# raphaelsulzer/PixelsPointsPolygons

Measured on AMD Instinct MI355X. Metric: training tiles/sec (224px img + 3k-pt lidar), higher is better.
Workload: dtype f32 (products as bf16x3 on the bf16 MFMA, fp32 accumulate); 1 GPU; pix2poly_fusion_s8_bs64x1; tiles_per_gpu=64, points_per_tile=3000, hip_graph=True, sync_bn=False, decoder_dropout=reference defaults (0.1 / 0.05), step=fwd+CE+10*BCE+bwd+AdamW, parallelism=dp1

## Files before the change

### include/p3hip.h

```cpp
#ifndef P3HIP_H
#define P3HIP_H
#include <stdint.h>

#ifdef __cplusplus
extern "C" {
#endif

#define P3_OK 0
#define P3_EINVAL (-1)
#define P3_ESHAPE (-2)
#define P3_EALIGN (-3)
#define P3_EUNSUP (-4)

#define P3_F32 0
#define P3_BF16 1
#define P3_F32X3 2

#define P3_ACT_NONE 0
#define P3_ACT_GELU 1
#define P3_ACT_RELU 2
#define P3_ACT_MUL 3
#define P3_ACT_BN_RELU 4

#define P3_A_PLAIN 0
// ... 217 lines not shown
int p3_gemm_tn(const void* A, const void* B, float* C, int M, int N, int K, int lda, int ldb, int ldc, int dtype, void* stream);
int p3_colsum(const void* x, float* out, int64_t M, int N, int ld, int dtype, void* stream);
int p3_act_bwd(const void* dy, int dtype_dy, const void* saved, int dtype_saved, void* out, int dtype_out, int64_t n, int act, float scale,
               void* stream);
int p3_embed_tokens_bwd(const void* dx, int dtype, const int64_t* tokens, float* demb, float* dpos, int B, int L, int D, void* stream);
int p3_embed_tokens_bwd_v(const void* dx, int dtype, const int64_t* tokens, float* demb, int B, int L, int D, int V, void* stream);
int p3_tokens_assemble_bwd(const float* dx, const void* src, int src_ld, int dtype_src, const float* scale, const float* shift, const float* mean,
                           void* dsrc, float* dscale, float* dshift, int B, int np, int D, void* stream);
int p3_pool_pos_bwd(const void* dout, int dtype_dout, void* dy, int dtype_dy, int B, int np, int Din, int Dout, void* stream);
int p3_pair_mean_bwd(const float* dF, void* dfeats, int dtype, int B, int L, int N, int D, int accumulate, void* stream);
int p3_sinkhorn_bwd(const float* scores, const float* alpha, int B, int m, int n, int iters, const float* perm,
                    const float* uv_hist, const float* dperm, float* dscores, float* dalpha, void* workspace, void* stream);
int64_t p3_sinkhorn_bwd_workspace_bytes(int B, int m, int n, int iters);
int p3_ce_loss_fwd(const float* logits, int ld, const int64_t* targets, int R, int V, int ignore_index, float* row_lse, float* acc, void* stream);
int p3_ce_loss_bwd(const float* logits, int ld, const int64_t* targets, int R, int V, int ignore_index, const float* row_lse,
                   const float* acc, const float* gscale, void* dlogits, int dtype_out, int ld_out, int Vpad, void* stream);
int p3_bce_loss_fwd(const float* p, const float* y, int64_t n, float* acc, void* stream);
int p3_bce_loss_bwd(const float* p, const float* y, int64_t n, const float* gscale, float* dp, void* stream);
int p3_adamw_schedule(long long* step, float* hyper, float base_lr, int kind, int warmup_steps, int total_steps, float beta1, float beta2,
                      void* stream);
int p3_adamw_schedule_dev(long long* step, float* hyper, const float* sched, float beta1, float beta2, void* stream);
int p3_adamw(float* params, const float* grads, float* exp_avg, float* exp_avg_sq, int64_t n, const float* hyper, float beta1,
             float beta2, float eps, float weight_decay, float grad_scale, void* bf16_shadow, void* stream);

int p3_gemm_tn_ex(const void* A, const void* B, float* C, int M, int N, int K, int lda, int ldb, int ldc, int dtype, int b_mode,
                  const float* b_scale, const float* b_shift, const void* pair_V, int pair_n, float* colsum ,
                  float* slabs ,
                  int max_slabs, void* stream);
int p3_row_affine_bwd(const void* dA, const float* dS, const void* H, const float* scale, const float* shift, const float* mean, const float* w4,
                      void* dHd, float* acc, int64_t R, int C, int N, int transpose, int dtype, void* stream);
int p3_row_affine_bwd2(const void* dA, const float* dS, const void* H, const float* scale, const float* shift, const float* mean,
                       const float* w4, void* dHd, float* acc, const float* fix_a, const float* fix_b, int64_t R, int C, int N,
                       int transpose, int dtype, void* stream);
int p3_bn_bwd_coeffs(const float* dscale, const float* dshift, const float* gamma, const float* mean, const float* rstd, float count,
                     int training, int C, float* dgamma, float* dbeta, float* a, float* b, void* stream);
int p3_affine_fix(void* dH, const void* H, const float* a, const float* b, int64_t R, int C, int dtype, void* stream);
int p3_affine_fix_ld(void* dH, const void* H, int ldh, const float* a, const float* b, int64_t R, int C, int dtype, void* stream);
int p3_pair_bwd(const void* dA, const void* U, const void* V, const float* scale, const float* shift, const float* mean, float* dU, float* dV, float* acc,
                int B, int N, int C, int dtype, void* stream);
int64_t p3_pair_bwd_workspace_bytes(int B, int N, int C);
int64_t p3_pair_bwd_workspace_bytes_dt(int B, int N, int C, int dtype);
int p3_pair_bwd_ws(const void* dA, const void* U, const void* V, const float* scale, const float* shift, const float* mean, float* dU, float* dV,
                   float* acc, int B, int N, int C, int dtype, void* workspace, void* stream);
int p3_bn_sums_from_g(const float* G, int ldg, const float* W, const float* scale, const float* shift, const float* mean, float* dW, float* acc,
                      int N, int K, void* stream);
int64_t p3_pair_bwd_fused_workspace_bytes(int B, int N);
int p3_pair_bwd_fused(const void* dH2, const void* W2t, const void* U, const void* V, const float* scale, const float* shift, const float* mean,
                      float* dU, float* dV, float* acc, int B, int N, void* workspace, void* stream);
int p3_pair_stats_bwd(const void* U, const void* V, const float* a, const float* b, float* dU, float* dV, int B, int N, int C, int dtype,
                      void* stream);
int p3_pair_bwd_fused_x3(const float* dH2, const float* W2t, const float* U, const float* V, const float* scale, const float* shift, const float* mean,
                         float* dU, float* dV, float* acc, int B, int N, void* workspace, void* stream);

int p3_upsample_bilinear(const void* src, int dtype_src, void* dst, int dtype_dst, int B, int h, int w, int C, int H, int W, int ld,
                         int src_tok_off, int src_tok_per_img, void* stream);
int p3_head1x1(const void* X, int ld, int dtype, const float* scale, const float* shift, const float* W, const float* bias, int n_out,
               int act, float post_mul, float* out_nchw, void* copy_dst, int copy_ld, int64_t R, int64_t HW, void* stream);
int p3_nhwc_to_nchw(const void* X, int ld, int dtype, const float* scale, const float* shift, float* out, int B, int C, int64_t HW, void* stream);

int p3_head1x1_bwd(const void* H, int dtype, const float* scale, const float* shift, const float* mean, const float* W, int n_out,
                   const float* out_nchw, const float* dout_nchw, int act, float post_mul, void* dHd, float* acc, int64_t R, int64_t HW,
                   void* stream);
int p3_affine_relu_bwd256(const void* dA, const void* H, int ldh, int dtype, const float* scale, const float* shift, const float* mean,
                          void* dHd, float* acc, int64_t R, void* stream);
int p3_pad_nhwc(const void* src, int ld_src, int dtype, const float* scale, const float* shift, int c_aff, int C, int Cp, void* dst, int B, int H,
                int W, void* stream);
// ... 81 lines not shown
```

### pixelspointspolygons_amd/backward.py

```python
import torch

SUMS_FROM_G = [__import__("os").environ.get("P3_SUMS_FROM_G", "1") != "0"]
FUSED_BN2 = [__import__("os").environ.get("P3_BN2_FUSED", "1") != "0"]
FUSED_PAIR = [__import__("os").environ.get("P3_PAIR_FUSED", "1") != "0"]


def scorenet_backward(net, feats, keep, dout, transpose_acc):
    from . import ops
    return ops.drive_steps([scorenet_backward_steps(net, feats, keep, dout, transpose_acc)])[0]


def scorenet_backward_steps(net, feats, keep, dout, transpose_acc):
    from . import hip, ops
    cd, N, training = net.cd, net.n_vertices, net.training
    B, L, D = feats.shape
    dev = feats.device
    R = B * N * N
    F_, U, V, H2, H3 = keep["F"], keep["U"], keep["V"], keep["H2"], keep["H3"]
    (sc1, sh1, m1, r1), (sc2, sh2, m2, r2), (sc3, sh3, m3, r3) = keep["bn"]
    cnt = float(R)
    w2d = lambda conv: conv.weight.reshape(conv.weight.shape[0], -1)
    f32 = dict(dtype=torch.float32, device=dev)
    acc3 = torch.zeros(3 * 64 + 1, **f32)
    dS, w4 = dout.contiguous(), net.conv4.weight.detach().reshape(-1)
    dH3 = hip.row_affine_bwd(H3, sc3, sh3, m3, acc3, dS=dS, w4=w4, N=N, transpose=transpose_acc, store=not training)
    dw4, db4 = acc3[128:192].view(1, 64, 1, 1), acc3[192:193]
    dg3, dbt3, a3, b3 = yield from ops.bn_backward_coeffs_steps(acc3[:64], acc3[64:128], net.bn3.weight.detach(), m3, r3, cnt, training, params=(net.bn3.weight, net.bn3.bias))
    if training:
        dH3 = hip.row_affine_bwd(H3, sc3, sh3, m3, None, dS=dS, w4=w4, N=N, transpose=transpose_acc, fix=(a3, b3))
    gw = {n: ops.direct_grads(getattr(net, n).weight) for n in ("conv1", "conv2", "conv3")}
    wout = lambda n, r, c: gw[n][0].view(r, c) if gw[n] is not None else torch.zeros(r, c, **f32)
    db3 = ops.bias_grad_before_bn(dH3, training, net.conv3.bias)
    w3t = ops.shadow(net.conv3.weight, cd, key="2dT", fn=lambda t: t.reshape(t.shape[0], -1).t())
    acc2 = torch.zeros(2 * 128, **f32)
    fused2 = training and SUMS_FROM_G[0] and FUSED_BN2[0]
    dA3 = None if fused2 else hip.gemm(dH3, w3t, out_dtype=cd)
    if training and SUMS_FROM_G[0]:
        G = torch.zeros((64, 256), **f32)
        hip.gemm_tn_ex(dH3, H2, G, hip.A_AFFINE_MASK2, sc2, sh2)
        dW3 = wout("conv3", 64, 128)
        hip.bn_sums_from_g(G, net.conv3.weight.detach().reshape(64, 128), sc2, sh2, m2, dW3, acc2)
        dH2 = None
    else:
        dW3 = hip.gemm_tn_ex(dH3, H2, wout("conv3", 64, 128), hip.A_AFFINE_RELU, sc2, sh2)
        dH2 = hip.row_affine_bwd(H2, sc2, sh2, m2, acc2, dA=dA3, out=dA3, store=not training)
    dg2, dbt2, a2, b2 = yield from ops.bn_backward_coeffs_steps(acc2[:128], acc2[128:], net.bn2.weight.detach(), m2, r2, cnt, training, params=(net.bn2.weight, net.bn2.bias))
    if fused2:
        dH2 = hip.gemm(dH3, w3t, out_dtype=cd, bwd=(H2, hip.ACT_BN_RELU, torch.stack([sc2, sh2, a2, b2])))
    elif training:
        dH2 = hip.row_affine_bwd(H2, sc2, sh2, m2, None, dA=dA3, out=dA3, fix=(a2, b2))
    dW2 = hip.gemm_tn_ex(dH2, U, wout("conv2", 128, 256), hip.A_PAIR_AFFINE_RELU, sc1, sh1, pair_v=V, pair_n=N, M=R)
    db2 = ops.bias_grad_before_bn(dH2, training, net.conv2.bias)
    w2t = ops.shadow(net.conv2.weight, cd, key="2dT", fn=lambda t: t.reshape(t.shape[0], -1).t())
    acc1 = torch.zeros(2 * 256, **f32)
    if (cd == torch.bfloat16 or (cd == torch.float32 and hip.split_now())) and FUSED_PAIR[0]:
        dU, dV = hip.pair_bwd_fused(dH2, w2t, U, V, sc1, sh1, m1, B, N, acc1)
    else:
        dA2 = hip.gemm(dH2, w2t, out_dtype=cd)
        dU, dV = hip.pair_bwd(dA2, U, V, sc1, sh1, m1, B, N, acc1)
    dg1, dbt1, a1, b1 = yield from ops.bn_backward_coeffs_steps(acc1[:256], acc1[256:], net.bn1.weight.detach(), m1, r1, cnt, training, params=(net.bn1.weight, net.bn1.bias))
    if training:
        hip.pair_stats_bwd(U, V, a1, b1, dU, dV, B, N)
    dUc, dVc = hip.cast(dU, cd), hip.cast(dV, cd)
    F2 = F_.view(B * N, D)
    dW1 = wout("conv1", 256, 2 * D)
    hip.gemm_tn(dUc, F2, out=dW1[:, :D])
    hip.gemm_tn(dVc, F2, out=dW1[:, D:])
    db1 = ops.bias_grad_before_bn(dU, training, net.conv1.bias)
    w1t = ops.shadow(net.conv1.weight, cd, key="2dT2", fn=lambda t: torch.cat([t.reshape(256, -1)[:, :D].t(), t.reshape(256, -1)[:, D:].t()], 0))
    dF = hip.gemm(dUc, w1t[:D], out_dtype=torch.float32)
    dF = hip.gemm(dVc, w1t[D:], out_dtype=torch.float32, residual=dF)
    dfeats = hip.pair_mean_bwd(dF, B, L, N, D, feats.dtype)
    wret = lambda n, t, shape: None if gw[n] is not None else t.view(*shape)
    if any(v is not None for v in gw.values()):
        ops._grad_ready(*(getattr(net, n).weight for n in gw if gw[n] is not None))
    grads = {"conv1.weight": wret("conv1", dW1, (256, 2 * D, 1, 1)), "conv1.bias": db1, "bn1.weight": dg1, "bn1.bias": dbt1,
             "conv2.weight": wret("conv2", dW2, (128, 256, 1, 1)), "conv2.bias": db2, "bn2.weight": dg2, "bn2.bias": dbt2,
             "conv3.weight": wret("conv3", dW3, (64, 128, 1, 1)), "conv3.bias": db3, "bn3.weight": dg3, "bn3.bias": dbt3,
             "conv4.weight": dw4, "conv4.bias": db4}
    return dfeats, [grads[n] for n, _ in net.named_parameters()]
```

### pixelspointspolygons_amd/csrc/mask2_dw_x3.hip

```cpp
#include <stdlib.h>

#include "p3_common.h"

namespace {

constexpr int MX_ROWS = 64;
constexpr int MX_A = MX_ROWS * 128, MX_B = MX_ROWS * 256;
constexpr int MX_OFF_AL = MX_A, MX_OFF_M1 = 2 * MX_A, MX_OFF_M2H = MX_OFF_M1 + MX_B, MX_OFF_M2L = MX_OFF_M2H + MX_B;
constexpr int MX_STEP = MX_OFF_M2L + MX_B;
constexpr int MX_LDS = 2 * MX_STEP;

struct MxArgs {
    const float* dH; const float* H2; const float* sc; const float* sh;
    float* C; int ldc; float* slabs; int64_t steps;
};

__global__ __launch_bounds__(512, 2) void mask2_dw_x3_kernel(MxArgs g) {
    extern __shared__ __attribute__((aligned(1024))) unsigned char lds[];
    const int tid = threadIdx.x, lane = tid & 63, wave = __builtin_amdgcn_readfirstlane(tid >> 6), l31 = lane & 31;
    const int mi = wave & 1, nq = wave >> 1;
    const uint32_t lds_addr = __builtin_amdgcn_readfirstlane((uint32_t)(uintptr_t)lds);
    const int64_t my_steps = (g.steps - (int64_t)blockIdx.x + (int64_t)gridDim.x - 1) / (int64_t)gridDim.x;
    const int ar = tid >> 3, ack = tid & 7, bck = tid & 15;
    float scv[8], shv[8];
#pragma unroll
    for (int e = 0; e < 8; ++e) { scv[e] = g.sc[bck * 8 + e]; shv[e] = g.sh[bck * 8 + e]; }
    float4 pa[2], pb[2][2];
    auto fetch = [&](int64_t q) __attribute__((always_inline)) {
        const int64_t row0 = ((int64_t)blockIdx.x + q * (int64_t)gridDim.x) * MX_ROWS;
        const float* ap = g.dH + (row0 + ar) * 64 + ack * 8;
        pa[0] = *reinterpret_cast<const float4*>(ap); pa[1] = *reinterpret_cast<const float4*>(ap + 4);
#pragma unroll
        for (int k = 0; k < 2; ++k) {
            const float* bp = g.H2 + (row0 + k * 32 + (tid >> 4)) * 128 + bck * 8;
            pb[k][0] = *reinterpret_cast<const float4*>(bp); pb[k][1] = *reinterpret_cast<const float4*>(bp + 4);
        }
    };
    auto commit = [&](int buf) __attribute__((always_inline)) {
        unsigned char* base = lds + buf * MX_STEP;
        {
            const float x[8] = {pa[0].x, pa[0].y, pa[0].z, pa[0].w, pa[1].x, pa[1].y, pa[1].z, pa[1].w};
            u32x4_t h, l;
            split8(x, h, l);
            const uint32_t off = (uint32_t)(ar * 128 + ((ack ^ (((ar >> 1) & 1) << 2)) * 16));
            *reinterpret_cast<u32x4_t*>(base + off) = h;
            *reinterpret_cast<u32x4_t*>(base + MX_OFF_AL + off) = l;
        }
#pragma unroll
        for (int k = 0; k < 2; ++k) {
            const int r = k * 32 + (tid >> 4);
            const float x[8] = {pb[k][0].x, pb[k][0].y, pb[k][0].z, pb[k][0].w, pb[k][1].x, pb[k][1].y, pb[k][1].z, pb[k][1].w};
            float m[8];
            u32x4_t m1;
#pragma unroll
            for (int e = 0; e < 4; ++e) {
                const bool on0 = fmaf(x[2 * e], scv[2 * e], shv[2 * e]) > 0.f, on1 = fmaf(x[2 * e + 1], scv[2 * e + 1], shv[2 * e + 1]) > 0.f;
                m1[e] = (on0 ? 0x3f80u : 0u) | (on1 ? 0x3f800000u : 0u);
                m[2 * e] = on0 ? x[2 * e] : 0.f; m[2 * e + 1] = on1 ? x[2 * e + 1] : 0.f;
            }
            u32x4_t h, l;
            split8(m, h, l);
            const uint32_t off = (uint32_t)(r * 256 + ((bck ^ ((r & 3) << 2)) * 16));
            *reinterpret_cast<u32x4_t*>(base + MX_OFF_M1 + off) = m1;
            *reinterpret_cast<u32x4_t*>(base + MX_OFF_M2H + off) = h;
            *reinterpret_cast<u32x4_t*>(base + MX_OFF_M2L + off) = l;
        }
    };
    f32x16 acc[2];
#pragma unroll
    for (int k = 0; k < 2; ++k)
#pragma unroll
        for (int r = 0; r < 16; ++r) acc[k][r] = 0.f;
    const int g4 = lane >> 4, li = lane & 15;
    uint32_t offa[2], offb[2];
#pragma unroll
    for (int hh = 0; hh < 2; ++hh) {
        const int row = (g4 >> 1) * 8 + hh * 4 + (li >> 2);
        const int sa = mi * 4 + (g4 & 1) * 2 + ((li & 3) >> 1), sb = nq * 4 + (g4 & 1) * 2 + ((li & 3) >> 1);
        offa[hh] = (uint32_t)(row * 128 + ((sa ^ (((row >> 1) & 1) << 2)) * 16) + ((li & 3) & 1) * 8);
        offb[hh] = (uint32_t)(row * 256 + ((sb ^ ((row & 3) << 2)) * 16) + ((li & 3) & 1) * 8);
    }
    if (my_steps > 0) { fetch(0); commit(0); }
    for (int64_t q = 0; q < my_steps; ++q) {
        __syncthreads();
        if (q + 1 < my_steps) fetch(q + 1);
        __builtin_amdgcn_sched_barrier(0);
        const uint32_t base = lds_addr + (uint32_t)((q & 1) * MX_STEP);
#pragma unroll
        for (int kk = 0; kk < MX_ROWS / 16; ++kk) {
            u32x2_t fah[2], fal[2], f1[2], f2h[2], f2l[2];
#pragma unroll
            for (int hh = 0; hh < 2; ++hh) {
                const uint32_t oa = base + (uint32_t)(kk * 16 * 128) + offa[hh], ob = base + (uint32_t)(kk * 16 * 256) + offb[hh];
                lds_read_tr16_b64(fah[hh], oa);
                lds_read_tr16_b64(fal[hh], oa + (uint32_t)MX_OFF_AL);
                lds_read_tr16_b64(f1[hh], ob + (uint32_t)MX_OFF_M1);
                lds_read_tr16_b64(f2h[hh], ob + (uint32_t)MX_OFF_M2H);
                lds_read_tr16_b64(f2l[hh], ob + (uint32_t)MX_OFF_M2L);
            }
            asm volatile("s_waitcnt lgkmcnt(0)" : "+v"(fah[0]), "+v"(fah[1]), "+v"(fal[0]), "+v"(fal[1]), "+v"(f1[0]), "+v"(f1[1]), "+v"(f2h[0]), "+v"(f2h[1]),
                                                  "+v"(f2l[0]), "+v"(f2l[1]));
            auto frag = [](const u32x2_t (&f)[2]) __attribute__((always_inline)) { return __builtin_bit_cast(bf16x8_t, u32x4_t{f[0].x, f[0].y, f[1].x, f[1].y}); };
            const bf16x8_t ah = frag(fah), al = frag(fal), m1 = frag(f1), m2h = frag(f2h), m2l = frag(f2l);
            acc[0] = __builtin_amdgcn_mfma_f32_32x32x16_bf16(al, m1, acc[0], 0, 0, 0);
            acc[0] = __builtin_amdgcn_mfma_f32_32x32x16_bf16(ah, m1, acc[0], 0, 0, 0);
            acc[1] = __builtin_amdgcn_mfma_f32_32x32x16_bf16(al, m2h, acc[1], 0, 0, 0);
            acc[1] = __builtin_amdgcn_mfma_f32_32x32x16_bf16(ah, m2l, acc[1], 0, 0, 0);
            acc[1] = __builtin_amdgcn_mfma_f32_32x32x16_bf16(ah, m2h, acc[1], 0, 0, 0);
        }
        if (q + 1 < my_steps) commit((int)((q + 1) & 1));
    }
    const int hi = lane >> 5;
#pragma unroll
    for (int k = 0; k < 2; ++k) {
        const int c = k * 128 + nq * 32 + l31;
#pragma unroll
        for (int r = 0; r < 16; ++r) {
            const int n = mi * 32 + crow32(r, hi);
            if (g.slabs) g.slabs[((int64_t)blockIdx.x * 64 + n) * 256 + c] = acc[k][r];
            else atomicAdd(g.C + (int64_t)n * g.ldc + c, acc[k][r]);
        }
    }
}

}

int p3_mask2_dw_x3_try(const void* A, const void* B, float* C, int M, int N, int Kb, int lda, int ldb, int ldc, const float* scale, const float* shift,
                       float* slabs, int max_slabs, hipStream_t s) {
    if (N != 64 || Kb != 128 || lda != 64 || ldb != 128 || M % MX_ROWS != 0 || M < MX_ROWS * 256) return P3_SKIP;
    if ((((uintptr_t)A | (uintptr_t)B) % 16) != 0) return P3_SKIP;
    MxArgs g;
    g.dH = (const float*)A; g.H2 = (const float*)B; g.sc = scale; g.sh = shift; g.C = C; g.ldc = ldc; g.steps = M / MX_ROWS;
    const int grid = 256;
    g.slabs = (slabs && grid <= max_slabs) ? slabs : nullptr;
    const int rc = p3_launch<mask2_dw_x3_kernel>("mask2_dw_x3_kernel", dim3(grid), dim3(512), MX_LDS, s, g);
    if (rc != P3_OK) return rc;
    if (g.slabs) p3_tn_reduce_launch(g.slabs, C, 64, 256, ldc, grid, s);
    return P3_OK;
}
```

### pixelspointspolygons_amd/csrc/rows_x3.hip

```cpp
#include "p3_common.h"

namespace {

struct RXArgs {
    const float* X;
    const float* W;
    float* Y;
    const float* bias;
    const float* a_scale;
    const float* a_shift;
    float* stats;
    int64_t groups;
};

__global__ __launch_bounds__(256, 2) void rows_x3_fwd_kernel(RXArgs g) {
    constexpr int K = 128, N = 64;
    __shared__ float tab[2 * K];
    __shared__ float red[2][2 * N];
    const int tid = threadIdx.x, lane = tid & 63, w = tid >> 6, l32 = lane & 31, hi = lane >> 5;
    const int nb = w & 1, stream = w >> 1;
    for (int i = tid; i < K; i += 256) { tab[i] = g.a_scale[i]; tab[K + i] = g.a_shift[i]; }
    __syncthreads();
    const int ch = nb * 32 + l32;
    bf16x8_t wh[8], wl[8];
#pragma unroll
    for (int s = 0; s < 8; ++s) {
        const float* wp = g.W + (int64_t)ch * K + 16 * s + 8 * hi;
        const float4 x0 = *reinterpret_cast<const float4*>(wp), x1 = *reinterpret_cast<const float4*>(wp + 4);
        const float v[8] = {x0.x, x0.y, x0.z, x0.w, x1.x, x1.y, x1.z, x1.w};
        u32x4_t h, l;
        split8(v, h, l);
        wh[s] = __builtin_bit_cast(bf16x8_t, h); wl[s] = __builtin_bit_cast(bf16x8_t, l);
    }
// ... 21 lines not shown
            split8(a, ah_, al_);
            const bf16x8_t ah = __builtin_bit_cast(bf16x8_t, ah_), al = __builtin_bit_cast(bf16x8_t, al_);
            const int ks = half * 4 + s;
            acc = __builtin_amdgcn_mfma_f32_32x32x16_bf16(al, wh[ks], acc, 0, 0, 0);
            acc = __builtin_amdgcn_mfma_f32_32x32x16_bf16(ah, wl[ks], acc, 0, 0, 0);
            acc = __builtin_amdgcn_mfma_f32_32x32x16_bf16(ah, wh[ks], acc, 0, 0, 0);
            __builtin_amdgcn_sched_barrier(0);
        }
    };
    if (gi < g.groups) fetch(xa, gi, 0);
    for (; gi < g.groups; gi += nw) {
        fetch(xb, gi, 1);
#pragma unroll
        for (int r = 0; r < 16; ++r) acc[r] = 0.f;
        mma_half(xa, 0);
        if (gi + nw < g.groups) fetch(xa, gi + nw, 0);
        mma_half(xb, 1);
        float* yp = g.Y + (gi * 32 + 4 * hi) * N + ch;
#pragma unroll
        for (int r = 0; r < 16; ++r) {
            const float v = acc[r] + bias;
            s1 += v; s2 = fmaf(v, v, s2);
            yp[((r & 3) + 8 * (r >> 2)) * N] = v;
        }
    }
    if (g.stats) {
        const float a1 = s1 + __shfl_xor(s1, 32, 64), a2 = s2 + __shfl_xor(s2, 32, 64);
        if (hi == 0) { red[stream][ch] = a1; red[stream][N + ch] = a2; }
        __syncthreads();
        if (tid < 2 * N) g.stats[(int64_t)blockIdx.x * 2 * N + tid] = red[0][tid] + red[1][tid];
    }
}

}

int p3_rows_x3_try(const void* A, const void* W, void* C, const p3_gemm_desc* d, hipStream_t s) {
    if (d->dtype_in != P3_F32 || d->dtype_out != P3_F32 || d->M % 32 != 0 || d->M < 4096) return P3_SKIP;
    if (d->a_mode != P3_A_AFFINE_RELU || d->K != 128 || d->N != 64 || d->bwd_saved) return P3_SKIP;
    if (d->lda != d->K || d->ldb != d->K || d->ldc != d->N) return P3_SKIP;
    if (d->act != P3_ACT_NONE || d->residual || d->aux || (d->drop.seed && d->drop.p > 0.f)) return P3_SKIP;
    if (((uintptr_t)A | (uintptr_t)W | (uintptr_t)C) % 16 != 0) return P3_SKIP;
    RXArgs g;
    g.X = (const float*)A; g.W = (const float*)W; g.Y = (float*)C; g.bias = d->bias; g.a_scale = d->a_scale; g.a_shift = d->a_shift; g.stats = nullptr;
    g.groups = d->M / 32;
    int64_t blocks = (g.groups + 1) / 2;
    if (blocks > 512) blocks = 512;
    float* scratch = nullptr;
    if (d->colsum) {
        const int nch = (int)((blocks + 127) / 128);
        scratch = p3_reduce_scratch(blocks * 128 + (int64_t)nch * 128);
        if (!scratch) return P3_SKIP;
        g.stats = scratch;
    }
    const int rc = p3_launch<rows_x3_fwd_kernel>("rows_x3_fwd_kernel", dim3((unsigned)blocks), dim3(256), 0, s, g);
    if (rc != P3_OK) return rc;
    if (scratch) return p3_det_reduce2(scratch, (int)blocks, 128, scratch + blocks * 128, d->colsum, d->colsumsq, 64, 128, 1, s);
    return P3_OK;
}
```

### pixelspointspolygons_amd/csrc/scorenet_bwd.hip

```cpp
#include <stdlib.h>

#include "p3_common.h"

namespace {

template <typename T>
__device__ __forceinline__ void ld4(const T* p, float (&v)[4]) {
    if constexpr (sizeof(T) == 2) {
        const uint2 raw = *reinterpret_cast<const uint2*>(p);
        v[0] = __uint_as_float(raw.x << 16); v[1] = __uint_as_float(raw.x & 0xffff0000u);
        v[2] = __uint_as_float(raw.y << 16); v[3] = __uint_as_float(raw.y & 0xffff0000u);
    } else {
        const float4 raw = *reinterpret_cast<const float4*>(p);
        v[0] = raw.x; v[1] = raw.y; v[2] = raw.z; v[3] = raw.w;
    }
}
template <typename T>
__device__ __forceinline__ void st4(T* p, const float (&v)[4]) {
    if constexpr (sizeof(T) == 2) {
        uint2 raw; raw.x = pack_bf2(v[0], v[1]); raw.y = pack_bf2(v[2], v[3]);
        *reinterpret_cast<uint2*>(p) = raw;
    } else {
        *reinterpret_cast<float4*>(p) = make_float4(v[0], v[1], v[2], v[3]);
    }
}

template <typename T, int C, bool TAIL>
__global__ __launch_bounds__(256) void row_affine_bwd_kernel(const T* __restrict__ dA, const float* __restrict__ dS, const T* __restrict__ H,
                                                             const float* __restrict__ sc, const float* __restrict__ sh, const float* __restrict__ mean,
                                                             const float* __restrict__ w4, T* __restrict__ dHd, float* __restrict__ acc,
                                                             int64_t R, int N, int transpose, const float* __restrict__ fix_a,
                                                             const float* __restrict__ fix_b, float* __restrict__ slab) {
    constexpr int LPR = C / 4, RPW = 64 / LPR;
    const int lane = threadIdx.x & 63, sub = lane % LPR, rsel = lane / LPR, w = threadIdx.x >> 6;
    const int c0 = sub * 4;
    float s[4], h[4], wv[4], mu[4];
#pragma unroll
    for (int k = 0; k < 4; ++k) { s[k] = sc[c0 + k]; h[k] = sh[c0 + k]; mu[k] = mean[c0 + k]; wv[k] = TAIL ? w4[c0 + k] : 0.f; }
    float a_sc[4] = {0, 0, 0, 0}, a_sh[4] = {0, 0, 0, 0}, a_w[4] = {0, 0, 0, 0}, a_b = 0.f;
    float fa[4] = {0, 0, 0, 0}, fb[4] = {0, 0, 0, 0};
    if (fix_a) {
#pragma unroll
        for (int k = 0; k < 4; ++k) { fa[k] = fix_a[c0 + k]; fb[k] = fix_b[c0 + k]; }
    }
    const int64_t wave_id = (int64_t)blockIdx.x * 4 + w, nwaves = (int64_t)gridDim.x * 4;
    constexpr int UNR = TAIL ? 4 : 1;
    for (int64_t r0 = wave_id * RPW; r0 < R; r0 += nwaves * RPW * UNR) {
        float hv[UNR][4], g[UNR][4], gr[UNR];
        bool ok[UNR];
#pragma unroll
        for (int u = 0; u < UNR; ++u) {
            const int64_t r = r0 + (int64_t)u * nwaves * RPW + rsel;
            ok[u] = r < R;
            const int64_t rc = ok[u] ? r : R - 1;
            ld4<T>(H + rc * C + c0, hv[u]);
            gr[u] = 0.f;
            if constexpr (TAIL) {
                int64_t rs = rc;
                if (transpose) { const int64_t nn = (int64_t)N * N, b = rc / nn, p = rc - b * nn; const int i = (int)(p / N), j = (int)(p - (int64_t)i * N); rs = b * nn + (int64_t)j * N + i; }
                gr[u] = dS[rs];
            } else {
                ld4<T>(dA + rc * C + c0, g[u]);
            }
        }
#pragma unroll
        for (int u = 0; u < UNR; ++u) {
            if (!ok[u]) continue;
            const int64_t r = r0 + (int64_t)u * nwaves * RPW + rsel;
            if constexpr (TAIL) {
                if (sub == 0) a_b += gr[u];
#pragma unroll
                for (int k = 0; k < 4; ++k) { g[u][k] = gr[u] * wv[k]; a_w[k] += gr[u] * fmaxf(hv[u][k] * s[k] + h[k], 0.f); }
            }
            float o[4];
#pragma unroll
            for (int k = 0; k < 4; ++k) {
                const float dz = (hv[u][k] * s[k] + h[k] > 0.f) ? g[u][k] : 0.f;
                a_sc[k] += dz * (hv[u][k] - mu[k]); a_sh[k] += dz;
                o[k] = dz * s[k] + fa[k] + fb[k] * hv[u][k];
            }
            if (dHd) st4<T>(dHd + r * C + c0, o);
        }
    }
    if (!acc) return;
#pragma unroll
    for (int o = LPR; o < 64; o <<= 1) {
#pragma unroll
        for (int k = 0; k < 4; ++k) { a_sc[k] += __shfl_xor(a_sc[k], o, 64); a_sh[k] += __shfl_xor(a_sh[k], o, 64); if (TAIL) a_w[k] += __shfl_xor(a_w[k], o, 64); }
        if (TAIL) a_b += __shfl_xor(a_b, o, 64);
    }
    __shared__ float red[4][3 * C + 1];
    if (rsel == 0) {
#pragma unroll
        for (int k = 0; k < 4; ++k) { red[w][c0 + k] = a_sc[k]; red[w][C + c0 + k] = a_sh[k]; red[w][2 * C + c0 + k] = a_w[k]; }
        if (sub == 0) red[w][3 * C] = a_b;
    }
    __syncthreads();
    const int nvals = TAIL ? 3 * C + 1 : 2 * C;
    for (int i = threadIdx.x; i < nvals; i += 256) {
        const float v = (red[0][i] + red[1][i]) + (red[2][i] + red[3][i]);
        if (slab) slab[(int64_t)blockIdx.x * nvals + i] = v;
        else atomicAdd(acc + i, v);
    }
}

__global__ void bn_bwd_coeffs_kernel(const float* __restrict__ dscale, const float* __restrict__ dshift, const float* __restrict__ gamma,
                                     const float* __restrict__ mean, const float* __restrict__ rstd, float count, int training, int C,
                                     float* __restrict__ dgamma, float* __restrict__ dbeta, float* __restrict__ a, float* __restrict__ b) {
    const int c = blockIdx.x * blockDim.x + threadIdx.x;
    if (c >= C) return;
    const float ds = dscale[c], dh = dshift[c], g = gamma[c], m = mean[c], rs = rstd[c];
    if (training & 2) { dgamma[c] += ds * rs; dbeta[c] += dh; }
// ... 396 lines not shown
```

### pixelspointspolygons_amd/hip.py

```python
import ctypes
import math
import os
from ctypes import Structure, byref, c_float, c_int, c_int64, c_void_p

import torch

from ._lib import P3Error, check, lib

F32, BF16, F32X3 = 0, 1, 2
ACT_NONE, ACT_GELU, ACT_RELU, ACT_MUL, ACT_BN_RELU = 0, 1, 2, 3, 4
A_PLAIN, A_CONV3X3, A_AFFINE_RELU, A_PAIR_AFFINE_RELU = 0, 1, 2, 3


class _KernelTimer:

    def __init__(self):
        self.on, self.pending = False, []

    def enable(self):
        self.on, self.pending = True, []
        lib().p3_trace_kernels(1)

    def disable(self):
        self.on = False
# ... 1443 lines not shown

def adamw_schedule(step, hyper, base_lr, kind, warmup, total, beta1, beta2):
    check(lib().p3_adamw_schedule(ptr(step), ptr(hyper), base_lr, kind, warmup, total, beta1, beta2, stream()), "p3_adamw_schedule")


def adamw_schedule_dev(step, hyper, sched, beta1, beta2):
    check(lib().p3_adamw_schedule_dev(ptr(step), ptr(hyper), ptr(sched), beta1, beta2, stream()), "p3_adamw_schedule_dev")


def adamw(params, grads, m, v, hyper, beta1, beta2, eps, wd, grad_scale=1.0, shadow=None):
    check(lib().p3_adamw(ptr(params), ptr(grads), ptr(m), ptr(v), params.numel(), ptr(hyper), beta1, beta2, eps, wd, grad_scale, ptr(shadow), stream()), "p3_adamw")


A_AFFINE_MASK2 = 5


def bn_sums_from_g(G, W, scale, shift, mean, dW, acc):
    N, K = W.shape
    check(lib().p3_bn_sums_from_g(ptr(G), G.stride(0), ptr(W), ptr(scale), ptr(shift), ptr(mean), ptr(dW), ptr(acc), N, K, stream()), "p3_bn_sums_from_g")


def gemm_tn_ex(a, b, out, b_mode, b_scale, b_shift, pair_v=None, pair_n=0, M=None):
    M_ = a.shape[0] if M is None else M
    N, K = a.shape[1], b.shape[1]
    if tuple(out.shape) != (N, K * (2 if b_mode == A_AFFINE_MASK2 else 1)) or out.dtype != torch.float32:
        raise P3Error(f"gemm_tn_ex: out must be float32 [{N}, {K * (2 if b_mode == A_AFFINE_MASK2 else 1)}], got {out.dtype} {tuple(out.shape)}")
    slabs, ns = _tn_slabs(N, K * (2 if b_mode == A_AFFINE_MASK2 else 1), a)
    check(lib().p3_gemm_tn_ex(ptr(a), ptr(b), ptr(out), M_, N, K, a.stride(0), b.stride(0),
                              out.stride(0), dt_mm(a), b_mode, ptr(b_scale), ptr(b_shift), ptr(pair_v), pair_n,
                              ptr(None), ptr(slabs), ns, stream()), "p3_gemm_tn_ex")
    return out


def row_affine_bwd(H, scale, shift, mean, acc, *, dA=None, dS=None, w4=None, N=0, transpose=False, out=None, store=True, fix=None):
    R, C = H.shape
    if store:
        out = out if out is not None else torch.empty_like(H)
    else:
        out = None
    fa, fb = fix if fix is not None else (None, None)
    check(lib().p3_row_affine_bwd2(ptr(dA), ptr(dS), ptr(H), ptr(scale), ptr(shift), ptr(mean), ptr(w4), ptr(out), ptr(acc), ptr(fa), ptr(fb),
                                   R, C, N, int(transpose), dt(H), stream()), "p3_row_affine_bwd")
    return out


def bn_bwd_coeffs(dscale, dshift, gamma, mean, rstd, count, training, acc=None):
    C = gamma.shape[0]
    o = torch.empty((4, C), dtype=torch.float32, device=gamma.device)
    dg, db = (acc[0], acc[1]) if acc is not None else (o[0], o[1])
    check(lib().p3_bn_bwd_coeffs(ptr(dscale), ptr(dshift), ptr(gamma), ptr(mean), ptr(rstd), count,
                                 int(bool(training)) | (2 if acc is not None else 0), C,
                                 ptr(dg), ptr(db), ptr(o[2]), ptr(o[3]), stream()), "p3_bn_bwd_coeffs")
    return (None, None, o[2], o[3]) if acc is not None else (o[0], o[1], o[2], o[3])


def affine_fix(dH, H, a, b, ldh=None):
    R, C = dH.shape
    check(lib().p3_affine_fix_ld(ptr(dH), ptr(H), ldh if ldh is not None else H.stride(0), ptr(a), ptr(b), R, C, dt(dH), stream()), "p3_affine_fix")
    return dH


def pair_bwd(dA, U, V, scale, shift, mean, B, N, acc):
    C = U.shape[1]
    dU = torch.empty((B * N, C), dtype=torch.float32, device=U.device)
    dV = torch.zeros((B * N, C), dtype=torch.float32, device=U.device)
    L = lib()
# ... 314 lines not shown
```

Before: 970.4 tiles/s.

## Recompute scorenet layer-3 gradient inside the dW3 and dH2 backward kernels

Stops materialising the conv3 pre-BN gradient dH3 (an R x 64 fp32 tensor). Its two consumers, the masked dW3 GEMM and the dH2 GEMM with fused BN-ReLU backward, now regenerate it per element from H3, dS and small per-channel tables held in LDS. This removes one full-size write-and-read pass over dH3 and one kernel launch. In exchange both kernels do extra elementwise work, read H3 twice, and gain a dedicated rows_x3 backward MFMA kernel for the K=64, N=128 case.

```diff
diff --git a/include/p3hip.h b/include/p3hip.h
--- a/include/p3hip.h
+++ b/include/p3hip.h
@@ -273,6 +273,11 @@
 int p3_row_affine_bwd2(const void* dA, const float* dS, const void* H, const float* scale, const float* shift, const float* mean,
                        const float* w4, void* dHd, float* acc, const float* fix_a, const float* fix_b, int64_t R, int C, int N,
                        int transpose, int dtype, void* stream);
+int p3_mask2_dw_x3_tail(const float* H3, const float* dS, const float* sc3, const float* sh3, const float* w4, const float* a3, const float* b3,
+                        const float* H2, const float* sc2, const float* sh2, float* G, int ldg, int64_t R, int N, int transpose, float* slabs,
+                        int max_slabs, void* stream);
+int p3_rows_x3_bwd_tail(const float* H3, const float* dS, const float* sc3, const float* sh3, const float* w4, const float* a3, const float* b3,
+                        const float* W3t, const float* H2, const float* bn2, float* dH2, int64_t R, int N, int transpose, void* stream);
 int p3_bn_bwd_coeffs(const float* dscale, const float* dshift, const float* gamma, const float* mean, const float* rstd, float count,
                      int training, int C, float* dgamma, float* dbeta, float* a, float* b, void* stream);
 int p3_affine_fix(void* dH, const void* H, const float* a, const float* b, int64_t R, int C, int dtype, void* stream);
diff --git a/pixelspointspolygons_amd/backward.py b/pixelspointspolygons_amd/backward.py
--- a/pixelspointspolygons_amd/backward.py
+++ b/pixelspointspolygons_amd/backward.py
@@ -2,6 +2,7 @@
 
 SUMS_FROM_G = [__import__("os").environ.get("P3_SUMS_FROM_G", "1") != "0"]
 FUSED_BN2 = [__import__("os").environ.get("P3_BN2_FUSED", "1") != "0"]
+TAIL_FUSED = [__import__("os").environ.get("P3_TAIL_FUSED", "1") != "0"]
 FUSED_PAIR = [__import__("os").environ.get("P3_PAIR_FUSED", "1") != "0"]
 
 
@@ -21,23 +22,28 @@
     cnt = float(R)
     w2d = lambda conv: conv.weight.reshape(conv.weight.shape[0], -1)
     f32 = dict(dtype=torch.float32, device=dev)
+    fused2 = training and SUMS_FROM_G[0] and FUSED_BN2[0]
+    tail_fused = fused2 and TAIL_FUSED[0] and hip.tail_fused_ok(H3)
     acc3 = torch.zeros(3 * 64 + 1, **f32)
     dS, w4 = dout.contiguous(), net.conv4.weight.detach().reshape(-1)
     dH3 = hip.row_affine_bwd(H3, sc3, sh3, m3, acc3, dS=dS, w4=w4, N=N, transpose=transpose_acc, store=not training)
     dw4, db4 = acc3[128:192].view(1, 64, 1, 1), acc3[192:193]
     dg3, dbt3, a3, b3 = yield from ops.bn_backward_coeffs_steps(acc3[:64], acc3[64:128], net.bn3.weight.detach(), m3, r3, cnt, training, params=(net.bn3.weight, net.bn3.bias))
-    if training:
+    if training and not tail_fused:
         dH3 = hip.row_affine_bwd(H3, sc3, sh3, m3, None, dS=dS, w4=w4, N=N, transpose=transpose_acc, fix=(a3, b3))
+    tail = (sc3, sh3, w4, a3, b3)
     gw = {n: ops.direct_grads(getattr(net, n).weight) for n in ("conv1", "conv2", "conv3")}
     wout = lambda n, r, c: gw[n][0].view(r, c) if gw[n] is not None else torch.zeros(r, c, **f32)
-    db3 = ops.bias_grad_before_bn(dH3, training, net.conv3.bias)
+    db3 = ops.bias_grad_before_bn(H3 if tail_fused else dH3, training, net.conv3.bias)
     w3t = ops.shadow(net.conv3.weight, cd, key="2dT", fn=lambda t: t.reshape(t.shape[0], -1).t())
     acc2 = torch.zeros(2 * 128, **f32)
-    fused2 = training and SUMS_FROM_G[0] and FUSED_BN2[0]
     dA3 = None if fused2 else hip.gemm(dH3, w3t, out_dtype=cd)
     if training and SUMS_FROM_G[0]:
         G = torch.zeros((64, 256), **f32)
-        hip.gemm_tn_ex(dH3, H2, G, hip.A_AFFINE_MASK2, sc2, sh2)
+        if tail_fused:
+            hip.mask2_dw_x3_tail(H3, dS, tail, H2, sc2, sh2, G, N, transpose_acc)
+        else:
+            hip.gemm_tn_ex(dH3, H2, G, hip.A_AFFINE_MASK2, sc2, sh2)
         dW3 = wout("conv3", 64, 128)
         hip.bn_sums_from_g(G, net.conv3.weight.detach().reshape(64, 128), sc2, sh2, m2, dW3, acc2)
         dH2 = None
@@ -46,7 +52,8 @@
         dH2 = hip.row_affine_bwd(H2, sc2, sh2, m2, acc2, dA=dA3, out=dA3, store=not training)
     dg2, dbt2, a2, b2 = yield from ops.bn_backward_coeffs_steps(acc2[:128], acc2[128:], net.bn2.weight.detach(), m2, r2, cnt, training, params=(net.bn2.weight, net.bn2.bias))
     if fused2:
-        dH2 = hip.gemm(dH3, w3t, out_dtype=cd, bwd=(H2, hip.ACT_BN_RELU, torch.stack([sc2, sh2, a2, b2])))
+        bn2 = torch.stack([sc2, sh2, a2, b2])
+        dH2 = hip.rows_x3_bwd_tail(H3, dS, tail, w3t, H2, bn2, N, transpose_acc) if tail_fused else hip.gemm(dH3, w3t, out_dtype=cd, bwd=(H2, hip.ACT_BN_RELU, bn2))
     elif training:
         dH2 = hip.row_affine_bwd(H2, sc2, sh2, m2, None, dA=dA3, out=dA3, fix=(a2, b2))
     dW2 = hip.gemm_tn_ex(dH2, U, wout("conv2", 128, 256), hip.A_PAIR_AFFINE_RELU, sc1, sh1, pair_v=V, pair_n=N, M=R)
diff --git a/pixelspointspolygons_amd/csrc/mask2_dw_x3.hip b/pixelspointspolygons_amd/csrc/mask2_dw_x3.hip
--- a/pixelspointspolygons_amd/csrc/mask2_dw_x3.hip
+++ b/pixelspointspolygons_amd/csrc/mask2_dw_x3.hip
@@ -1,6 +1,7 @@
 #include <stdlib.h>
 
 #include "p3_common.h"
+#include "scorenet_tail.h"
 
 namespace {
 
@@ -13,10 +14,14 @@
 struct MxArgs {
     const float* dH; const float* H2; const float* sc; const float* sh;
     float* C; int ldc; float* slabs; int64_t steps;
+    ScoreTail t;
 };
 
-__global__ __launch_bounds__(512, 2) void mask2_dw_x3_kernel(MxArgs g) {
+template <bool GEN>
+__device__ __forceinline__ void mask2_dw_x3_body(const MxArgs& g) {
     extern __shared__ __attribute__((aligned(1024))) unsigned char lds[];
+    __shared__ __attribute__((aligned(16))) float tab[GEN ? ST_FLOATS : 4];
+    if constexpr (GEN) scorenet_tail_tables(tab, g.t, (int)threadIdx.x, 512);
     const int tid = threadIdx.x, lane = tid & 63, wave = __builtin_amdgcn_readfirstlane(tid >> 6), l31 = lane & 31;
     const int mi = wave & 1, nq = wave >> 1;
     const uint32_t lds_addr = __builtin_amdgcn_readfirstlane((uint32_t)(uintptr_t)lds);
@@ -26,10 +31,13 @@
 #pragma unroll
     for (int e = 0; e < 8; ++e) { scv[e] = g.sc[bck * 8 + e]; shv[e] = g.sh[bck * 8 + e]; }
     float4 pa[2], pb[2][2];
+    float pds = 0.f;
+    const float* asrc = GEN ? g.t.H3 : g.dH;
     auto fetch = [&](int64_t q) __attribute__((always_inline)) {
         const int64_t row0 = ((int64_t)blockIdx.x + q * (int64_t)gridDim.x) * MX_ROWS;
-        const float* ap = g.dH + (row0 + ar) * 64 + ack * 8;
+        const float* ap = asrc + (row0 + ar) * 64 + ack * 8;
         pa[0] = *reinterpret_cast<const float4*>(ap); pa[1] = *reinterpret_cast<const float4*>(ap + 4);
+        if constexpr (GEN) pds = g.t.dS[scorenet_tail_ds_index(row0 + ar, g.t.N, g.t.transpose)];
 #pragma unroll
         for (int k = 0; k < 2; ++k) {
             const float* bp = g.H2 + (row0 + k * 32 + (tid >> 4)) * 128 + bck * 8;
@@ -39,7 +47,13 @@
     auto commit = [&](int buf) __attribute__((always_inline)) {
         unsigned char* base = lds + buf * MX_STEP;
         {
-            const float x[8] = {pa[0].x, pa[0].y, pa[0].z, pa[0].w, pa[1].x, pa[1].y, pa[1].z, pa[1].w};
+            const float x0[8] = {pa[0].x, pa[0].y, pa[0].z, pa[0].w, pa[1].x, pa[1].y, pa[1].z, pa[1].w};
+            float x[8];
+            if constexpr (GEN) scorenet_tail_grad8(tab, ack * 8, pds, x0, x);
+            else {
+#pragma unroll
+                for (int e = 0; e < 8; ++e) x[e] = x0[e];
+            }
             u32x4_t h, l;
             split8(x, h, l);
             const uint32_t off = (uint32_t)(ar * 128 + ((ack ^ (((ar >> 1) & 1) << 2)) * 16));
@@ -80,6 +94,7 @@
         offa[hh] = (uint32_t)(row * 128 + ((sa ^ (((row >> 1) & 1) << 2)) * 16) + ((li & 3) & 1) * 8);
         offb[hh] = (uint32_t)(row * 256 + ((sb ^ ((row & 3) << 2)) * 16) + ((li & 3) & 1) * 8);
     }
+    if constexpr (GEN) __syncthreads();
     if (my_steps > 0) { fetch(0); commit(0); }
     for (int64_t q = 0; q < my_steps; ++q) {
         __syncthreads();
@@ -123,6 +138,20 @@
     }
 }
 
+__global__ __launch_bounds__(512, 2) void mask2_dw_x3_kernel(MxArgs g) { mask2_dw_x3_body<false>(g); }
+__global__ __launch_bounds__(512, 2) void mask2_dw_x3_tail_kernel(MxArgs g) { mask2_dw_x3_body<true>(g); }
+
+int mask2_launch(MxArgs& g, bool gen, float* C, int ldc, float* slabs, int max_slabs, hipStream_t s) {
+    const int grid = 256;
+    g.C = C; g.ldc = ldc;
+    g.slabs = (slabs && grid <= max_slabs) ? slabs : nullptr;
+    const int rc = gen ? p3_launch<mask2_dw_x3_tail_kernel>("mask2_dw_x3_tail_kernel", dim3(grid), dim3(512), MX_LDS, s, g)
+                       : p3_launch<mask2_dw_x3_kernel>("mask2_dw_x3_kernel", dim3(grid), dim3(512), MX_LDS, s, g);
+    if (rc != P3_OK) return rc;
+    if (g.slabs) p3_tn_reduce_launch(g.slabs, C, 64, 256, ldc, grid, s);
+    return P3_OK;
+}
+
 }
 
 int p3_mask2_dw_x3_try(const void* A, const void* B, float* C, int M, int N, int Kb, int lda, int ldb, int ldc, const float* scale, const float* shift,
@@ -130,11 +159,21 @@
     if (N != 64 || Kb != 128 || lda != 64 || ldb != 128 || M % MX_ROWS != 0 || M < MX_ROWS * 256) return P3_SKIP;
     if ((((uintptr_t)A | (uintptr_t)B) % 16) != 0) return P3_SKIP;
     MxArgs g;
-    g.dH = (const float*)A; g.H2 = (const float*)B; g.sc = scale; g.sh = shift; g.C = C; g.ldc = ldc; g.steps = M / MX_ROWS;
-    const int grid = 256;
-    g.slabs = (slabs && grid <= max_slabs) ? slabs : nullptr;
-    const int rc = p3_launch<mask2_dw_x3_kernel>("mask2_dw_x3_kernel", dim3(grid), dim3(512), MX_LDS, s, g);
-    if (rc != P3_OK) return rc;
-    if (g.slabs) p3_tn_reduce_launch(g.slabs, C, 64, 256, ldc, grid, s);
-    return P3_OK;
+    memset(&g, 0, sizeof(g));
+    g.dH = (const float*)A; g.H2 = (const float*)B; g.sc = scale; g.sh = shift; g.steps = M / MX_ROWS;
+    return mask2_launch(g, false, C, ldc, slabs, max_slabs, s);
 }
+
+extern "C" int p3_mask2_dw_x3_tail(const float* H3, const float* dS, const float* sc3, const float* sh3, const float* w4, const float* a3, const float* b3,
+                                   const float* H2, const float* sc2, const float* sh2, float* G, int ldg, int64_t R, int N, int transpose, float* slabs,
+                                   int max_slabs, void* stream) {
+    P3_CHECK(H3 && dS && sc3 && sh3 && w4 && a3 && b3 && H2 && sc2 && sh2 && G && R > 0 && N > 0 && ldg >= 256, P3_EINVAL, "p3_mask2_dw_x3_tail: bad arguments");
+    P3_CHECK(R % ((int64_t)N * N) == 0, P3_ESHAPE, "p3_mask2_dw_x3_tail: R == B*N*N");
+    P3_CHECK(R % MX_ROWS == 0 && R >= MX_ROWS * 256, P3_EUNSUP, "p3_mask2_dw_x3_tail: R % 64 == 0, R >= 16384");
+    P3_CHECK((((uintptr_t)H3 | (uintptr_t)H2) % 16) == 0, P3_EALIGN, "p3_mask2_dw_x3_tail: 16-byte base alignment");
+    MxArgs g;
+    memset(&g, 0, sizeof(g));
+    g.H2 = H2; g.sc = sc2; g.sh = sh2; g.steps = R / MX_ROWS;
+    g.t.H3 = H3; g.t.dS = dS; g.t.sc3 = sc3; g.t.sh3 = sh3; g.t.w4 = w4; g.t.a3 = a3; g.t.b3 = b3; g.t.N = N; g.t.transpose = transpose;
+    return mask2_launch(g, true, G, ldg, slabs, max_slabs, (hipStream_t)stream);
+}
diff --git a/pixelspointspolygons_amd/csrc/rows_x3.hip b/pixelspointspolygons_amd/csrc/rows_x3.hip
--- a/pixelspointspolygons_amd/csrc/rows_x3.hip
+++ b/pixelspointspolygons_amd/csrc/rows_x3.hip
@@ -1,4 +1,5 @@
 #include "p3_common.h"
+#include "scorenet_tail.h"
 
 namespace {
 
@@ -86,14 +87,111 @@
     }
 }
 
+struct RXBArgs {
+    const float* A;
+    const float* W;
+    const float* H2;
+    float* Y;
+    const float* bn;
+    ScoreTail t;
+    int64_t groups;
+};
+
+template <bool GEN>
+__global__ __launch_bounds__(256, 2) void rows_x3_bwd_kernel(RXBArgs g) {
+    constexpr int K = 64, N = 128;
+    __shared__ __attribute__((aligned(16))) float tab[GEN ? ST_FLOATS : 4];
+    const int tid = threadIdx.x, lane = tid & 63, w = tid >> 6, l32 = lane & 31, hi = lane >> 5;
+    if constexpr (GEN) { scorenet_tail_tables(tab, g.t, tid, 256); __syncthreads(); }
+    const int ch = w * 32 + l32;
+    bf16x8_t wh[4], wl[4];
+#pragma unroll
+    for (int s = 0; s < 4; ++s) {
+        const float* wp = g.W + (int64_t)ch * K + 16 * s + 8 * hi;
+        const float4 x0 = *reinterpret_cast<const float4*>(wp), x1 = *reinterpret_cast<const float4*>(wp + 4);
+        const float v[8] = {x0.x, x0.y, x0.z, x0.w, x1.x, x1.y, x1.z, x1.w};
+        u32x4_t h, l;
+        split8(v, h, l);
+        wh[s] = __builtin_bit_cast(bf16x8_t, h); wl[s] = __builtin_bit_cast(bf16x8_t, l);
+    }
+    const float bsc = g.bn[ch], bsh = g.bn[N + ch], ba = g.bn[2 * N + ch], bb = g.bn[3 * N + ch];
+    const float* src = GEN ? g.t.H3 : g.A;
+    const int64_t nw = gridDim.x;
+    int64_t gi = blockIdx.x;
+    float4 xa[4][2], xb[4][2];
+    float dsa = 0.f, dsb = 0.f;
+    auto fetch = [&](float4 (&x)[4][2], float& ds, int64_t grp) __attribute__((always_inline)) {
+        const int64_t row = grp * 32 + l32;
+        const float* xp = src + row * K + 8 * hi;
+#pragma unroll
+        for (int s = 0; s < 4; ++s) { x[s][0] = *reinterpret_cast<const float4*>(xp + 16 * s); x[s][1] = *reinterpret_cast<const float4*>(xp + 16 * s + 4); }
+        if constexpr (GEN) ds = g.t.dS[scorenet_tail_ds_index(row, g.t.N, g.t.transpose)];
+    };
+    auto step = [&](const float4 (&x)[4][2], const float ds, float4 (&xn)[4][2], float& dsn, int64_t grp) __attribute__((always_inline)) {
+        const float* hp = g.H2 + (grp * 32 + 4 * hi) * N + ch;
+        float hv[16];
+#pragma unroll
+        for (int r = 0; r < 16; ++r) hv[r] = hp[((r & 3) + 8 * (r >> 2)) * N];
+        if (grp + nw < g.groups) fetch(xn, dsn, grp + nw);
+        __builtin_amdgcn_sched_barrier(0);
+        f32x16 acc;
+#pragma unroll
+        for (int r = 0; r < 16; ++r) acc[r] = 0.f;
+#pragma unroll
+        for (int s = 0; s < 4; ++s) {
+            const float v[8] = {x[s][0].x, x[s][0].y, x[s][0].z, x[s][0].w, x[s][1].x, x[s][1].y, x[s][1].z, x[s][1].w};
+            float a[8];
+            if constexpr (GEN) scorenet_tail_grad8(tab, 16 * s + 8 * hi, ds, v, a);
+            else {
+#pragma unroll
+                for (int e = 0; e < 8; ++e) a[e] = v[e];
+            }
+            u32x4_t ah_, al_;
+            split8(a, ah_, al_);
+            const bf16x8_t ah = __builtin_bit_cast(bf16x8_t, ah_), al = __builtin_bit_cast(bf16x8_t, al_);
+            acc = __builtin_amdgcn_mfma_f32_32x32x16_bf16(al, wh[s], acc, 0, 0, 0);
+            acc = __builtin_amdgcn_mfma_f32_32x32x16_bf16(ah, wl[s], acc, 0, 0, 0);
+            acc = __builtin_amdgcn_mfma_f32_32x32x16_bf16(ah, wh[s], acc, 0, 0, 0);
+            __builtin_amdgcn_sched_barrier(0);
+        }
+        float* yp = g.Y + (grp * 32 + 4 * hi) * N + ch;
+#pragma unroll
+        for (int r = 0; r < 16; ++r) {
+            const float d = fmaf(hv[r], bsc, bsh) > 0.f ? __fmul_rn(acc[r], bsc) : 0.f;
+            yp[((r & 3) + 8 * (r >> 2)) * N] = fmaf(bb, hv[r], __fadd_rn(d, ba));
+        }
+    };
+    if (gi < g.groups) fetch(xa, dsa, gi);
+    while (gi < g.groups) {
+        step(xa, dsa, xb, dsb, gi);
+        gi += nw;
+        if (gi >= g.groups) break;
+        step(xb, dsb, xa, dsa, gi);
+        gi += nw;
+    }
+}
+
+template <bool GEN>
+int rows_x3_bwd_launch(RXBArgs& g, hipStream_t s) {
+    const int64_t blocks = g.groups < 512 ? g.groups : 512;
+    return p3_launch<rows_x3_bwd_kernel<GEN>>(GEN ? "rows_x3_bwd_kernel<true>" : "rows_x3_bwd_kernel<false>", dim3((unsigned)blocks), dim3(256), 0, s, g);
+}
+
 }
 
 int p3_rows_x3_try(const void* A, const void* W, void* C, const p3_gemm_desc* d, hipStream_t s) {
     if (d->dtype_in != P3_F32 || d->dtype_out != P3_F32 || d->M % 32 != 0 || d->M < 4096) return P3_SKIP;
-    if (d->a_mode != P3_A_AFFINE_RELU || d->K != 128 || d->N != 64 || d->bwd_saved) return P3_SKIP;
     if (d->lda != d->K || d->ldb != d->K || d->ldc != d->N) return P3_SKIP;
     if (d->act != P3_ACT_NONE || d->residual || d->aux || (d->drop.seed && d->drop.p > 0.f)) return P3_SKIP;
     if (((uintptr_t)A | (uintptr_t)W | (uintptr_t)C) % 16 != 0) return P3_SKIP;
+    if (d->a_mode == P3_A_PLAIN && d->K == 64 && d->N == 128 && d->bwd_saved && d->bwd_act == P3_ACT_BN_RELU && !d->bias && !d->colsum &&
+        (uintptr_t)d->bwd_saved % 16 == 0) {
+        RXBArgs b;
+        memset(&b, 0, sizeof(b));
+        b.A = (const float*)A; b.W = (const float*)W; b.H2 = (const float*)d->bwd_saved; b.Y = (float*)C; b.bn = d->bwd_bn; b.groups = d->M / 32;
+        return rows_x3_bwd_launch<false>(b, s);
+    }
+    if (d->a_mode != P3_A_AFFINE_RELU || d->K != 128 || d->N != 64 || d->bwd_saved) return P3_SKIP;
     RXArgs g;
     g.X = (const float*)A; g.W = (const float*)W; g.Y = (float*)C; g.bias = d->bias; g.a_scale = d->a_scale; g.a_shift = d->a_shift; g.stats = nullptr;
     g.groups = d->M / 32;
@@ -111,3 +209,16 @@
     if (scratch) return p3_det_reduce2(scratch, (int)blocks, 128, scratch + blocks * 128, d->colsum, d->colsumsq, 64, 128, 1, s);
     return P3_OK;
 }
+
+extern "C" int p3_rows_x3_bwd_tail(const float* H3, const float* dS, const float* sc3, const float* sh3, const float* w4, const float* a3, const float* b3,
+                                   const float* W3t, const float* H2, const float* bn2, float* dH2, int64_t R, int N, int transpose, void* stream) {
+    P3_CHECK(H3 && dS && sc3 && sh3 && w4 && a3 && b3 && W3t && H2 && bn2 && dH2 && R > 0 && N > 0, P3_EINVAL, "p3_rows_x3_bwd_tail: bad arguments");
+    P3_CHECK(R % ((int64_t)N * N) == 0, P3_ESHAPE, "p3_rows_x3_bwd_tail: R == B*N*N");
+    P3_CHECK(R % 32 == 0 && R >= 4096, P3_EUNSUP, "p3_rows_x3_bwd_tail: R % 32 == 0, R >= 4096");
+    P3_CHECK((((uintptr_t)H3 | (uintptr_t)W3t | (uintptr_t)H2 | (uintptr_t)dH2) % 16) == 0, P3_EALIGN, "p3_rows_x3_bwd_tail: 16-byte base alignment");
+    RXBArgs b;
+    memset(&b, 0, sizeof(b));
+    b.W = W3t; b.H2 = H2; b.Y = dH2; b.bn = bn2; b.groups = R / 32;
+    b.t.H3 = H3; b.t.dS = dS; b.t.sc3 = sc3; b.t.sh3 = sh3; b.t.w4 = w4; b.t.a3 = a3; b.t.b3 = b3; b.t.N = N; b.t.transpose = transpose;
+    return rows_x3_bwd_launch<true>(b, (hipStream_t)stream);
+}
diff --git a/pixelspointspolygons_amd/csrc/scorenet_bwd.hip b/pixelspointspolygons_amd/csrc/scorenet_bwd.hip
--- a/pixelspointspolygons_amd/csrc/scorenet_bwd.hip
+++ b/pixelspointspolygons_amd/csrc/scorenet_bwd.hip
@@ -1,6 +1,7 @@
 #include <stdlib.h>
 
 #include "p3_common.h"
+#include "scorenet_tail.h"
 
 namespace {
 
@@ -56,9 +57,7 @@
             ld4<T>(H + rc * C + c0, hv[u]);
             gr[u] = 0.f;
             if constexpr (TAIL) {
-                int64_t rs = rc;
-                if (transpose) { const int64_t nn = (int64_t)N * N, b = rc / nn, p = rc - b * nn; const int i = (int)(p / N), j = (int)(p - (int64_t)i * N); rs = b * nn + (int64_t)j * N + i; }
-                gr[u] = dS[rs];
+                gr[u] = dS[scorenet_tail_ds_index(rc, N, transpose)];
             } else {
                 ld4<T>(dA + rc * C + c0, g[u]);
             }
@@ -70,14 +69,17 @@
             if constexpr (TAIL) {
                 if (sub == 0) a_b += gr[u];
 #pragma unroll
-                for (int k = 0; k < 4; ++k) { g[u][k] = gr[u] * wv[k]; a_w[k] += gr[u] * fmaxf(hv[u][k] * s[k] + h[k], 0.f); }
+                for (int k = 0; k < 4; ++k) a_w[k] += gr[u] * fmaxf(hv[u][k] * s[k] + h[k], 0.f);
             }
             float o[4];
 #pragma unroll
             for (int k = 0; k < 4; ++k) {
-                const float dz = (hv[u][k] * s[k] + h[k] > 0.f) ? g[u][k] : 0.f;
+                float dz;
+                if constexpr (TAIL) dz = scorenet_tail_dz(hv[u][k], gr[u], wv[k], s[k], h[k]);
+                else dz = (hv[u][k] * s[k] + h[k] > 0.f) ? g[u][k] : 0.f;
                 a_sc[k] += dz * (hv[u][k] - mu[k]); a_sh[k] += dz;
-                o[k] = dz * s[k] + fa[k] + fb[k] * hv[u][k];
+                if constexpr (TAIL) o[k] = scorenet_tail_fix(dz, hv[u][k], s[k], fa[k], fb[k]);
+                else o[k] = dz * s[k] + fa[k] + fb[k] * hv[u][k];
             }
             if (dHd) st4<T>(dHd + r * C + c0, o);
         }
diff --git a/pixelspointspolygons_amd/csrc/scorenet_tail.h b/pixelspointspolygons_amd/csrc/scorenet_tail.h
--- /dev/null
+++ b/pixelspointspolygons_amd/csrc/scorenet_tail.h
@@ -0,0 +1,40 @@
+#pragma once
+#include <stdint.h>
+
+__device__ __forceinline__ float scorenet_tail_dz(float h3, float ds, float w4, float sc, float sh) {
+    return fmaf(h3, sc, sh) > 0.f ? __fmul_rn(ds, w4) : 0.f;
+}
+__device__ __forceinline__ float scorenet_tail_fix(float dz, float h3, float sc, float a, float b) { return fmaf(b, h3, fmaf(dz, sc, a)); }
+__device__ __forceinline__ float scorenet_tail_grad(float h3, float ds, float w4, float sc, float sh, float a, float b) {
+    return scorenet_tail_fix(scorenet_tail_dz(h3, ds, w4, sc, sh), h3, sc, a, b);
+}
+
+__device__ __forceinline__ int64_t scorenet_tail_ds_index(int64_t r, int N, int transpose) {
+    if (!transpose) return r;
+    const int64_t nn = (int64_t)N * N, b = r / nn, p = r - b * nn;
+    const int i = (int)(p / N), j = (int)(p - (int64_t)i * N);
+    return b * nn + (int64_t)j * N + i;
+}
+
+struct ScoreTail {
+    const float* H3;
+    const float* dS;
+    const float* sc3; const float* sh3; const float* w4; const float* a3; const float* b3;
+    int N, transpose;
+};
+enum { ST_SC = 0, ST_SH = 64, ST_W4 = 128, ST_A = 192, ST_B = 256, ST_FLOATS = 320 };
+__device__ __forceinline__ void scorenet_tail_tables(float* tab, const ScoreTail& t, int tid, int nthreads) {
+    for (int i = tid; i < 64; i += nthreads) {
+        tab[ST_SC + i] = t.sc3[i]; tab[ST_SH + i] = t.sh3[i]; tab[ST_W4 + i] = t.w4[i]; tab[ST_A + i] = t.a3[i]; tab[ST_B + i] = t.b3[i];
+    }
+}
+__device__ __forceinline__ void scorenet_tail_grad8(const float* tab, int c0, float ds, const float (&h3)[8], float (&out)[8]) {
+    float t[5][8];
+#pragma unroll
+    for (int q = 0; q < 5; ++q) {
+        const float4 x0 = *reinterpret_cast<const float4*>(tab + 64 * q + c0), x1 = *reinterpret_cast<const float4*>(tab + 64 * q + c0 + 4);
+        t[q][0] = x0.x; t[q][1] = x0.y; t[q][2] = x0.z; t[q][3] = x0.w; t[q][4] = x1.x; t[q][5] = x1.y; t[q][6] = x1.z; t[q][7] = x1.w;
+    }
+#pragma unroll
+    for (int e = 0; e < 8; ++e) out[e] = scorenet_tail_grad(h3[e], ds, t[2][e], t[0][e], t[1][e], t[3][e], t[4][e]);
+}
diff --git a/pixelspointspolygons_amd/hip.py b/pixelspointspolygons_amd/hip.py
--- a/pixelspointspolygons_amd/hip.py
+++ b/pixelspointspolygons_amd/hip.py
@@ -1499,6 +1499,40 @@
     return out
 
 
+def tail_fused_ok(H3):
+    R = H3.shape[0]
+    return H3.dtype == torch.float32 and _SPLIT[0] and H3.is_contiguous() and H3.shape[1] == 64 and R % 64 == 0 and R >= 16384
+
+
+def mask2_dw_x3_tail(H3, dS, tail, H2, sc2, sh2, G, N, transpose):
+    sc3, sh3, w4, a3, b3 = tail
+    if tuple(G.shape) != (64, 256) or G.dtype != torch.float32:
+        raise P3Error(f"mask2_dw_x3_tail: G must be float32 [64, 256], got {G.dtype} {tuple(G.shape)}")
+    if H2.stride(0) != 128:
+        raise P3Error("mask2_dw_x3_tail: H2 is dense [R, 128]")
+    slabs, ns = _tn_slabs(64, 256, H3)
+    check(lib().p3_mask2_dw_x3_tail(ptr(H3), ptr(dS), ptr(sc3), ptr(sh3), ptr(w4), ptr(a3), ptr(b3), ptr(H2), ptr(sc2), ptr(sh2), ptr(G), G.stride(0),
+                                    H3.shape[0], N, int(transpose), ptr(slabs), ns, stream()), "p3_mask2_dw_x3_tail")
+    return G
+
+
+def rows_x3_bwd_tail(H3, dS, tail, w3t, H2, bn2, N, transpose, out=None):
+    sc3, sh3, w4, a3, b3 = tail
+    R = H3.shape[0]
+    if bn2.dtype != torch.float32 or tuple(bn2.shape) != (4, 128) or not bn2.is_contiguous() or tuple(w3t.shape) != (128, 64) or not w3t.is_contiguous():
+        raise P3Error("rows_x3_bwd_tail: needs a contiguous float32 [4, 128] table and a contiguous [128, 64] weight")
+    if out is None:
+        out = torch.empty((R, 128), dtype=torch.float32, device=H3.device)
+    if out.stride(0) != 128 or H2.stride(0) != 128 or tuple(out.shape) != (R, 128) or out.dtype != torch.float32:
+        raise P3Error("rows_x3_bwd_tail: H2 and out are dense float32 [R, 128]")
+    ev = KTIMER.begin()
+    check(lib().p3_rows_x3_bwd_tail(ptr(H3), ptr(dS), ptr(sc3), ptr(sh3), ptr(w4), ptr(a3), ptr(b3), ptr(w3t), ptr(H2), ptr(bn2), ptr(out), R, N,
+                                    int(transpose), stream()), "p3_rows_x3_bwd_tail")
+    if ev is not None:
+        KTIMER.end(ev, lib().p3_last_kernel().decode() or "rows_x3_bwd_kernel<true>", 2.0 * R * 128 * 64, float(R * (64 + 128 + 128) * 4))
+    return out
+
+
 def row_affine_bwd(H, scale, shift, mean, acc, *, dA=None, dS=None, w4=None, N=0, transpose=False, out=None, store=True, fix=None):
     R, C = H.shape
     if store:
```

Result: no change. 977.5 tiles/s (median of 6 runs) (+0.7%).
